# michaelneale/p2p-llm-tunnel

Measured on AMD Instinct MI355X. Metric: tunneled req/s + added p50 TTFT vs direct, mock-LLM SSE at 1/2/4/8 streams, higher is better.
Workload: dtype n/a

## Files before the change

### native/core/buf.h

```cpp
#pragma once

#include <atomic>
#include <cstdint>
#include <cstring>
#include <memory>
#include <string>
#include <string_view>
#include <vector>

namespace p2pt {

class Bytes {
 public:
  Bytes() = default;

  static Bytes copy(const void* p, size_t n) {
    auto v = std::make_shared<std::vector<uint8_t>>(static_cast<const uint8_t*>(p),
                                                    static_cast<const uint8_t*>(p) + n);
    return Bytes(std::move(v));
  }
  static Bytes copy(std::string_view s) { return copy(s.data(), s.size()); }
  static Bytes take(std::vector<uint8_t>&& v) {
    return Bytes(std::make_shared<std::vector<uint8_t>>(std::move(v)));
  }
// ... 61 lines not shown
    if (n < max_keep_) {
      bufs_.insert(bufs_.begin() + long(next_ < n ? next_ : n), b);
      next_ = next_ < n ? next_ + 1 : 0;
    }
    return b;
  }
  size_t size() const { return bufs_.size(); }

 private:
  static constexpr size_t kScan = 16;
  size_t size_, max_keep_;
  std::vector<RawBufPtr> bufs_;
  size_t next_ = 0;
};

inline Bytes slab_copy(const void* p, size_t n) {
  constexpr size_t kBlock = 64 * 1024, kMax = 2048;
  if (n == 0 || n > kMax) return Bytes::copy(p, n);
  struct Slab {
    BufPool pool{kBlock, 64};
    RawBufPtr cur;
    size_t off = kBlock;
  };
  thread_local Slab s;
  if (s.off + n > kBlock) {
    s.cur.reset();
    s.cur = s.pool.get();
    s.off = 0;
  }
  uint8_t* d = s.cur->data.get() + s.off;
  memcpy(d, p, n);
  s.off += (n + 15) & ~size_t(15);
  return Bytes::adopt(s.cur, d, n);
}

class ByteWriter {
 public:
  explicit ByteWriter(std::vector<uint8_t>& out) : out_(out) {}
  void u8(uint8_t v) { out_.push_back(v); }
  void u16(uint16_t v) {
    out_.push_back(uint8_t(v >> 8));
    out_.push_back(uint8_t(v));
  }
  void u32(uint32_t v) {
    out_.push_back(uint8_t(v >> 24));
    out_.push_back(uint8_t(v >> 16));
    out_.push_back(uint8_t(v >> 8));
    out_.push_back(uint8_t(v));
// ... 71 lines not shown
```

### native/http/client.cc

```cpp
#include "http/client.h"

#include "core/log.h"

#include <deque>

namespace p2pt::http {

using WarmWaiter = std::function<bool(std::shared_ptr<TcpConn>, const std::string&)>;

class ClientConnPool : public std::enable_shared_from_this<ClientConnPool> {
 public:
  explicit ClientConnPool(Reactor& r) : r_(r) {}
  std::shared_ptr<TcpConn> take(const std::string& key) {
    auto it = idle_.find(key);
    while (it != idle_.end() && !it->second.empty()) {
      auto c = it->second.back();
      it->second.pop_back();
      if (!c->closed()) return c;
    }
    return nullptr;
  }

  struct Warm {
    std::string host;
// ... 311 lines not shown
  live_calls()[this] = shared_from_this();
  pool_key_ = url_.scheme + "://" + url_.host + ":" + std::to_string(url_.port);
  pool_->call_started(pool_key_);
  counted_ = true;
  chunked_body_ = req_.stream_body && req_.content_length < 0;
  if (req_.stream_body) {
    for (auto& b : req_.body) queued_body_ += b.size();
    std::weak_ptr<ClientCall> w = shared_from_this();
    TcpConn::connect(*r_, url_.host, url_.port, url_.tls(), [w](std::shared_ptr<TcpConn> c, std::string e) {
      auto self = w.lock();
      if (!self || self->finished_) {
        if (c) c->close();
        return;
      }
      if (!c) {
        if (self->cb_.on_connect_failed) self->cb_.on_connect_failed();
        self->finish("error sending request for url (" + self->req_.url + "): " + e);
        return;
      }
      self->attach(c, false);
    });
    return;
  }
  if (auto c = pool_->take(pool_key_)) {
    attach(c, true);
    return;
  }
  if (auto c = pool_->take_warm(pool_key_)) {
    attach(c, true);
    return;
  }
  std::weak_ptr<ClientCall> w = shared_from_this();
  auto deliver = [w](std::shared_ptr<TcpConn> c, const std::string& e) -> bool {
    auto self = w.lock();
    if (!self || self->finished_) return false;
    if (!c) {
      if (self->cb_.on_connect_failed) self->cb_.on_connect_failed();
      self->finish("error sending request for url (" + self->req_.url + "): " + e);
      return true;
    }
    self->attach(c, false);
    return true;
  };
  if (pool_->wait_warm(pool_key_, deliver)) return;
  TcpConn::connect(*r_, url_.host, url_.port, url_.tls(), [deliver](std::shared_ptr<TcpConn> c, std::string e) {
    if (!deliver(c, e) && c) c->close();
  });
}

void ClientCall::attach(std::shared_ptr<TcpConn> c, bool reused) {
  conn_ = std::move(c);
  reused_ = reused;
  std::weak_ptr<ClientCall> w = shared_from_this();
  conn_->on_data([w](const uint8_t* p, size_t n) {
    if (auto s = w.lock()) s->on_data(p, n);
  });
  conn_->on_close([w](const std::string& err) {
    if (auto s = w.lock()) s->on_close(err);
  });
  std::string head;
  head.reserve(256);
  head += req_.method;
// ... 121 lines not shown

void ClientCall::on_close(const std::string& err) {
  auto self = shared_from_this();
  conn_.reset();
  if (finished_) return;
  if (!got_any_ && reused_) {
    reused_ = false;
    std::weak_ptr<ClientCall> w = self;
    TcpConn::connect(*r_, url_.host, url_.port, url_.tls(), [w](std::shared_ptr<TcpConn> c, std::string e) {
      auto s = w.lock();
      if (!s || s->finished_) {
        if (c) c->close();
        return;
      }
      if (!c) {
        if (s->cb_.on_connect_failed) s->cb_.on_connect_failed();
        s->finish("error sending request for url (" + s->req_.url + "): " + e);
        return;
      }
      s->attach(c, false);
    });
    return;
  }
  keep_alive_ = false;
  if (!head_done_) {
    process();
    if (finished_) return;
    finish("error sending request for url (" + req_.url + "): " +
           (err.empty() ? std::string("connection closed before message completed") : err));
    return;
  }
  paused_ = false;
// ... 92 lines not shown
```

### native/http/client.h

```cpp
#pragma once

#include <functional>
#include <map>
#include <memory>
#include <string>
#include <vector>

#include "core/net.h"
#include "http/http.h"

namespace p2pt::http {

struct ClientRequest {
  std::string method;
  std::string url;
  std::vector<Header> headers;
  std::vector<Bytes> body;
  uint64_t body_len = 0;
  bool force_content_length = false;
  bool stream_body = false;
  int64_t content_length = -1;
};

struct ClientCallbacks {
  std::function<void(bool reused)> on_sent;
  std::function<void(const Head&)> on_head;
  std::function<void(Bytes)> on_data;
  std::function<void(const std::string& err, bool before_head)> on_done;
  std::function<void()> on_connect_failed;
  std::function<void()> on_body_drain;
  size_t body_low_water = 64 * 1024;
};

class ClientConnPool;

class ClientCall : public std::enable_shared_from_this<ClientCall> {
 public:
  void pause();
  void resume();
  void cancel();
  bool finished() const { return finished_; }
  void write_body(Bytes b);
  void end_body();
  size_t body_backlog() const;
  ~ClientCall();

 private:
  friend class HttpClient;
  void start();
  void attach(std::shared_ptr<TcpConn> c, bool reused);
  void on_data(const uint8_t* p, size_t n);
  void on_close(const std::string& err);
  void finish(const std::string& err);
  void process();

  Reactor* r_ = nullptr;
  std::shared_ptr<ClientConnPool> pool_;
  ClientRequest req_;
  ClientCallbacks cb_;
  Url url_;
  std::string pool_key_;
  std::shared_ptr<TcpConn> conn_;
  bool reused_ = false;
  bool got_any_ = false;
  bool head_done_ = false;
  bool finished_ = false;
  bool paused_ = false;
  bool keep_alive_ = false;
// ... 27 lines not shown
```

### native/proto/frame.cc

```cpp
#include "proto/frame.h"

#include <algorithm>
#include <cstdlib>

#include <algorithm>
#include <cstring>

#include "core/crypto.h"

namespace p2pt::proto {

std::optional<MsgType> msg_type_from_u8(uint8_t v) {
  switch (v) {
    case 1: case 2: case 3: case 4:
    case 10: case 11: case 12: case 13: case 14: case 15:
    case 20: case 21: case 22:
    case 99:
      return MsgType(v);
    default:
      return std::nullopt;
  }
}

const char* msg_type_name(MsgType t) {
// ... 300 lines not shown
  }
  uint32_t st = 0;
  if (!get_u32(j, "stream_id", out.stream_id, err) || !get_u32(j, "status", st, err) ||
      !get_headers(j, out.headers, err))
    return false;
  if (st > 65535) {
    if (err) *err = "status out of range";
    return false;
  }
  out.status = uint16_t(st);
  return true;
}

Frame make_hello(const Hello& h) { return json_frame(MsgType::Hello, 0, h.to_json()); }
Frame make_agree(const Agree& a) { return json_frame(MsgType::Agree, 0, a.to_json()); }
Frame make_req_headers(const RequestHeaders& h) { return json_frame(MsgType::ReqHeaders, h.stream_id, h.to_json()); }
Frame make_res_headers(const ResponseHeaders& h) { return json_frame(MsgType::ResHeaders, h.stream_id, h.to_json()); }
Frame make_body(MsgType t, uint32_t sid, Bytes data) { return Frame{t, sid, std::move(data)}; }
Frame make_empty(MsgType t, uint32_t sid) { return Frame{t, sid, Bytes()}; }
Frame make_error(uint32_t sid, const std::string& msg) { return Frame{MsgType::Error, sid, Bytes::copy(msg)}; }
Frame make_credit(uint32_t sid, uint32_t bytes) {
  uint8_t b[4];
  wr32(b, bytes);
  return Frame{MsgType::Credit, sid, slab_copy(b, 4)};
}
uint32_t credit_bytes(const Frame& f) { return f.payload.size() == 4 ? rd32(f.payload.data()) : 0; }

static std::string trim_trailing_slashes(const std::string& s) {
  size_t n = s.size();
  while (n > 0 && s[n - 1] == '/') n--;
  return s.substr(0, n);
}
// ... 41 lines not shown
```

### native/proto/frame.h

```cpp
#pragma once

#include <cstdint>
#include <map>
#include <optional>
#include <string>
#include <vector>

#include "core/buf.h"
#include "core/json.h"

namespace p2pt::proto {

constexpr uint32_t kProtocolVersion = 1;
constexpr const char* kProtocolName = "httptunnel";
constexpr size_t kMaxFrameSize = 64 * 1024;
constexpr size_t kMaxBodyChunk = kMaxFrameSize - 128;
constexpr size_t kHeaderLen = 5;

enum class MsgType : uint8_t {
  Hello = 1,
  Agree = 2,
  Ping = 3,
  Pong = 4,
  ReqHeaders = 10,
// ... 69 lines not shown
  std::string method;
  std::string path;
  HeaderMap headers;
  Json to_json() const;
  static bool from_json(const Json& j, RequestHeaders& out, std::string* err);
};

struct ResponseHeaders {
  uint32_t stream_id = 0;
  uint16_t status = 200;
  HeaderMap headers;
  Json to_json() const;
  static bool from_json(const Json& j, ResponseHeaders& out, std::string* err);
};

Frame make_hello(const Hello& h);
Frame make_agree(const Agree& a);
Frame make_req_headers(const RequestHeaders& h);
Frame make_res_headers(const ResponseHeaders& h);
Frame make_body(MsgType t, uint32_t stream_id, Bytes data);
Frame make_empty(MsgType t, uint32_t stream_id);
Frame make_error(uint32_t stream_id, const std::string& msg);
Frame make_credit(uint32_t stream_id, uint32_t bytes);
uint32_t credit_bytes(const Frame& f);

constexpr int64_t kFlowWindow = 256 * 1024;
inline int64_t flow_window() { return kFlowWindow; }
constexpr size_t kFlowGrantMin = 16 * 1024;

constexpr int64_t kFlowMaxWindow = 8 * 1024 * 1024;
// ... 17 lines not shown
```

### native/py/module.cc

```cpp
#include <pybind11/pybind11.h>
#include <pybind11/stl.h>

#include "core/crypto.h"
#include "core/json.h"
#include "http/http.h"
#include "proto/frame.h"
#include "tunnel/app.h"
#include "ws/ws.h"

namespace py = pybind11;
using namespace p2pt;

static py::bytes to_py(const Bytes& b) { return py::bytes(reinterpret_cast<const char*>(b.data()), b.size()); }

static std::string canonical_json(const std::string& s) {
  Json j;
  std::string err;
  if (!Json::parse(s, j, &err)) throw py::value_error(err);
  return j.dump();
}

PYBIND11_MODULE(_native, m) {
  m.doc() = "p2p_llm_tunnel_amd native core";
  m.attr("MAX_FRAME_SIZE") = proto::kMaxFrameSize;
// ... 42 lines not shown
  });
  m.def("parse_request_headers", [](const std::string& s) {
    Json j;
    std::string err;
    proto::RequestHeaders h;
    if (!Json::parse(s, j, &err) || !proto::RequestHeaders::from_json(j, h, &err)) throw py::value_error(err);
    return py::make_tuple(h.stream_id, h.method, h.path, h.headers);
  });
  m.def("parse_response_headers", [](const std::string& s) {
    Json j;
    std::string err;
    proto::ResponseHeaders h;
    if (!Json::parse(s, j, &err) || !proto::ResponseHeaders::from_json(j, h, &err)) throw py::value_error(err);
    return py::make_tuple(h.stream_id, h.status, h.headers);
  });
  m.def("build_upstream_url", &proto::build_upstream_url);
  m.def("canonical_json", &canonical_json);
  m.def("crc32c", [](py::bytes b) {
    std::string s = b;
    return crc32c(s.data(), s.size());
  });
  m.def("crc32", [](py::bytes b) {
    std::string s = b;
    return crc32_ieee(s.data(), s.size());
  });
  m.def("ws_accept_key", [](const std::string& k) { return ws::accept_key(k); });
  m.def("ws_encode_frame", [](int op, py::bytes payload, bool mask) {
    std::string p = payload;
    return py::bytes(ws::encode_frame(ws::Op(op), p, mask));
  });
// ... 30 lines not shown
```

### native/tunnel/proxy.cc

```cpp
#include "tunnel/proxy.h"

#include <algorithm>
#include <cstdio>

#include "core/crypto.h"
#include "core/log.h"
#include "core/net.h"
#include "http/http.h"
#include "tunnel/assoc.h"
#include "tunnel/metrics.h"

namespace p2pt {

static const char* kT = "tunnel::proxy";

class ProxyWorker : public std::enable_shared_from_this<ProxyWorker> {
 public:
  ProxyWorker(Reactor& r, Reactor& assoc, std::weak_ptr<ProxySession> sess,
              std::shared_ptr<ProxySession::Shared> shared, size_t index)
      : r_(r), assoc_(assoc), sess_(std::move(sess)), shared_(std::move(shared)), index_(index) {}
  ~ProxyWorker();
  void init() {
    std::weak_ptr<ProxySession> w = sess_;
    size_t k = index_;
// ... 296 lines not shown
      body_.reset(mode, len);
      state_ = State::ReadingBody;
      reject_not_ready_ = true;
      if (body_.done()) finish_request_body();
      return true;
    }
    sid_ = sess->next_stream_id();
    metrics::counter_add("tunnel_streams_opened_total");
    trace::event("proxy", sid_, "accept");
    if (adopted_us_) {
      if (accepted_us_) trace::event_at("proxy", sid_, "tcp_accept", accepted_us_);
      trace::event_at("proxy", sid_, "conn_adopt", adopted_us_);
      accepted_us_ = adopted_us_ = 0;
    }
    if (req_.method == "GET") trace::event("proxy", sid_, "get");
    std::string path = req_.target;
    if (path.rfind("http://", 0) == 0 || path.rfind("https://", 0) == 0) {
      size_t s = path.find('/', path.find("://") + 3);
      path = s == std::string::npos ? "/" : path.substr(s);
    } else if (path == "*") {
      path = "/";
    }
    proto::RequestHeaders rh;
    rh.stream_id = sid_;
    rh.method = req_.method;
    rh.path = path;
    for (auto& hd : req_.headers)
      if (http::is_visible_ascii(hd.value)) proto::header_set(rh.headers, http::to_lower(hd.name), hd.value);
    LOG_DEBUG(kT, "proxying %s %s (stream %u)", rh.method.c_str(), rh.path.c_str(), sid_);
    proto::Frame hf = proto::make_req_headers(rh);
    if (hf.wire_size() > proto::kMaxFrameSize) {
      simple_and_close(431, "text/plain", "Request header fields too large for the tunnel");
      return false;
    }
    send_credit_ = proto::flow_window();
    credit_paused_ = false;
    owed_ = 0;
    rwin_ = proto::FlowWindow{};
    sess->register_stream(sid_, weak_from_this());
    stream_registered_ = true;
    sess->send(std::move(hf));
    if (req_.version_minor >= 1 && req_.has_token("expect", "100-continue"))
      conn_->write(std::string("HTTP/1.1 100 Continue\r\n\r\n"));
    body_.reset(mode, len);
    state_ = State::ReadingBody;
// ... 824 lines not shown
    }
    if (sched_->stream_queued(sid) <= cfg_.stream_budget / 4) {
      it->second.paused = false;
      p = paused_.erase(p);
      command(it->second.thread, Cmd{Cmd::Resume, sid});
      continue;
    }
    ++p;
  }
}

void ProxySession::route(const proto::Frame& f) {
  using proto::MsgType;
  switch (f.type) {
    case MsgType::ResHeaders: {
      Json j;
      std::string err;
      auto rh = std::make_shared<proto::ResponseHeaders>();
      if (!proto::json_parse_bytes(f.payload, j, &err) || !proto::ResponseHeaders::from_json(j, *rh, &err)) {
        LOG_ERROR(kT, "failed to parse response headers: %s", err.c_str());
        return;
      }
      LOG_DEBUG(kT, "response headers for stream %u: status=%u", rh->stream_id, rh->status);
      uint32_t sid = rh->stream_id;
      auto it = routes_.find(sid);
      if (it != routes_.end()) {
        Cmd c{Cmd::Headers, sid};
        c.urgent = true;
        c.rh = std::move(rh);
        command(it->second.thread, std::move(c));
      }
      break;
    }
    case MsgType::ResBody: {
// ... 181 lines not shown
```

### native/tunnel/serve.cc

```cpp
#include "tunnel/serve.h"

#include <algorithm>

#include "core/crypto.h"
#include "core/log.h"
#include "tunnel/assoc.h"
#include "tunnel/metrics.h"

namespace p2pt {

static const char* kT = "tunnel::serve";

class ServeWorker : public std::enable_shared_from_this<ServeWorker> {
 public:
  ServeWorker(Reactor& r, Reactor& assoc, std::weak_ptr<ServeSession> sess, const ServeConfig& cfg,
              std::vector<std::string> upstreams, bool is_inline)
      : r_(r), assoc_(assoc), sess_(std::move(sess)), cfg_(cfg), upstreams_(std::move(upstreams)),
        inline_(is_inline) {}

  ~ServeWorker() {
    auto calls = std::move(calls_);
    for (auto& kv : calls)
      if (kv.second.call) kv.second.call->cancel();
    client_.reset();
// ... 83 lines not shown
    if (f.type == proto::MsgType::ResBody && f.more.empty()) f.payload = out_->stage(f.payload);
    ev.frame = std::move(f);
    out_->push(std::move(ev), urgent);
  }

  void simple_response(uint32_t sid, uint16_t status, const std::string& body) {
    proto::ResponseHeaders rh;
    rh.stream_id = sid;
    rh.status = status;
    rh.headers.emplace_back("content-type", "text/plain");
    emit(sid, proto::make_res_headers(rh));
    emit(sid, proto::make_body(proto::MsgType::ResBody, sid, Bytes::copy(body)));
    emit(sid, proto::make_empty(proto::MsgType::ResEnd, sid));
  }

  void start(uint32_t sid, http::ClientRequest req, size_t body_chunk, bool retryable, bool grant) {
    if (!inline_) prewarm();
    std::weak_ptr<ServeWorker> w = shared_from_this();
    http::ClientCallbacks cb;
    if (req.stream_body) {
      cb.on_body_drain = [w, sid] {
        auto s = w.lock();
        if (!s) return;
        auto it = s->calls_.find(sid);
        if (it != s->calls_.end()) s->maybe_grant(sid, it->second);
      };
    }
    std::shared_ptr<ServeSession::Unreachable> back;
    if (retryable) {
      back = std::make_shared<ServeSession::Unreachable>();
      back->req = req;
    }
    auto unreachable = std::make_shared<bool>(false);
    cb.on_connect_failed = [unreachable] { *unreachable = true; };
    cb.on_sent = [sid](bool) { trace::event("serve", sid, "upstream_sent"); };
    cb.on_head = [w, sid](const http::Head& h) {
      auto s = w.lock();
      if (!s) return;
      proto::ResponseHeaders rh;
      rh.stream_id = sid;
      rh.status = uint16_t(h.status);
      for (auto& hd : h.headers)
        if (http::is_visible_ascii(hd.value)) proto::header_set(rh.headers, http::to_lower(hd.name), hd.value);
      s->emit(sid, proto::make_res_headers(rh), true);
      trace::event("serve", sid, "res_headers");
    };
    auto first = std::make_shared<bool>(true);
    size_t cs = body_chunk ? body_chunk : proto::kMaxBodyChunk;
    cb.on_data = [w, sid, first, cs](Bytes chunk) {
      auto s = w.lock();
      if (!s) return;
      const bool urgent = *first;
      if (*first) {
        *first = false;
        trace::event("serve", sid, "first_body");
      }
      size_t n = chunk.size();
      for (size_t off = 0; off < n; off += cs)
        s->emit(sid, proto::make_body(proto::MsgType::ResBody, sid, chunk.slice(off, cs)), urgent && off + cs >= n);
    };
    cb.on_done = [w, sid, back, unreachable](const std::string& err, bool before_head) {
      auto s = w.lock();
      if (!s) return;
      auto it = s->calls_.find(sid);
      if (it == s->calls_.end()) return;
      s->calls_.erase(it);
      ServeSession::Ev done(ServeSession::Ev::Done, sid);
      done.responded = !before_head;
      if (*unreachable && before_head) {
        if (back) {
          back->err = err;
          done.unreachable = back;
          s->out_->push(std::move(done));
          return;
        }
        done.unreachable = std::make_shared<ServeSession::Unreachable>();
        done.unreachable->err = err;
      }
      if (!err.empty() && before_head) {
        LOG_ERROR(kT, "upstream request failed: %s", err.c_str());
        metrics::counter_add("tunnel_upstream_errors_total");
        s->simple_response(sid, 502, "Bad Gateway: " + err);
      } else {
        if (!err.empty()) {
          LOG_ERROR(kT, "upstream stream error for stream %u: %s", sid, err.c_str());
          s->emit(sid, proto::make_error(sid, "upstream error: " + err));
        }
        s->emit(sid, proto::make_empty(proto::MsgType::ResEnd, sid));
        trace::event("serve", sid, "res_end");
        LOG_DEBUG(kT, "response %u complete", sid);
      }
      s->out_->push(std::move(done));
// ... 290 lines not shown
  sched_->send(proto::make_empty(proto::MsgType::Ping, 0));
  LOG_DEBUG(kT, "sent keepalive ping");
  std::weak_ptr<ServeSession> w = shared_from_this();
  ping_timer_ = r_.call_later_ms(cfg_.ping_interval_ms, [w] {
    if (auto s = w.lock()) {
      s->ping_timer_ = 0;
      s->send_ping();
    }
  });
}

void ServeSession::handle_frame(const proto::Frame& f) {
  using proto::MsgType;
  switch (f.type) {
    case MsgType::ReqHeaders: {
      Json j;
      std::string err;
      proto::RequestHeaders h;
      if (!proto::json_parse_bytes(f.payload, j, &err) || !proto::RequestHeaders::from_json(j, h, &err)) {
        LOG_WARN(kT, "malformed REQ_HEADERS for stream %u: %s", f.stream_id, err.c_str());
        send_simple_response(f.stream_id, 400, "Bad Request: malformed request headers");
        return;
      }
      LOG_DEBUG(kT, "request %u %s %s", h.stream_id, h.method.c_str(), h.path.c_str());
      trace::event("serve", h.stream_id, "req_headers");
      trace::rx_stamps("serve", h.stream_id);
      uint32_t sid = h.stream_id;
      Pending p;
      if (const std::string* cl = proto::header_get(h.headers, "content-length")) {
        char* end = nullptr;
        unsigned long long v = strtoull(cl->c_str(), &end, 10);
        if (end && *end == 0 && !cl->empty()) p.declared = int64_t(v);
      }
      p.headers = std::move(h);
// ... 184 lines not shown
  it->second.body_len = 0;
  send_simple_response(sid, 413, "Payload Too Large");
}

void ServeSession::start_request(uint32_t sid, Pending p, bool streaming) {
  if (!valid_method(p.headers.method)) {
    LOG_ERROR(kT, "failed to handle request: invalid HTTP method");
    send_simple_response(sid, 400, "Bad Request: invalid HTTP method");
    return;
  }
  if (inflight_.count(sid)) {
    LOG_WARN(kT, "stream %u reused while its response is in flight; ignoring the new request", sid);
    return;
  }
  http::ClientRequest req;
  req.method = p.headers.method;
  LOG_DEBUG(kT, "forwarding %s %s", p.headers.method.c_str(), p.headers.path.c_str());
  bool had_cl = false;
  for (auto& kv : p.headers.headers) {
    const std::string& k = kv.first;
    if (http::iequals(k, "host") || http::iequals(k, "connection") || http::iequals(k, "transfer-encoding"))
      continue;
    if (http::iequals(k, "content-length")) {
      had_cl = true;
      continue;
    }
    req.headers.push_back(http::Header{k, kv.second});
  }
  req.body = std::move(p.body);
  req.body_len = p.body_len;
  req.force_content_length = had_cl;
  if (streaming) {
    req.stream_body = true;
    req.content_length = p.declared;
  }
  metrics::counter_add("tunnel_upstream_requests_total");
  Inflight& fl = inflight_[sid];
  fl.up = pick_upstream();
  fl.route = BulkRoutes::key(req.method, p.headers.path);
  fl.thread = place_->pick(p.body_len >= Placement::kBulkBytes || p.declared >= int64_t(Placement::kBulkBytes) ||
                           bulk_routes_.bulk(fl.route));
  fl.path = std::move(p.headers.path);
// ... 108 lines not shown
```

Before: 15.97.

## Replace JSON tree header encode/decode with direct streaming codec

Adds a hand-written header codec that writes request/response header frames straight into a slab-allocated buffer and parses them without building a JSON tree. The proxy and serve paths switch to it, avoiding intermediate map and Json allocations per request. The serve worker's per-call callback state is merged into one shared context, and the retry copy of the request is now moved in only on connect failure rather than copied up front. Risks include subtle output differences versus the old JSON serializer in duplicate handling and escaping, plus a large new parser surface.

```diff
diff --git a/native/bin/headerbench_main.cc b/native/bin/headerbench_main.cc
--- /dev/null
+++ b/native/bin/headerbench_main.cc
@@ -0,0 +1,106 @@
+#include <algorithm>
+#include <chrono>
+#include <cstdio>
+#include <vector>
+
+#include "core/json.h"
+#include "http/http.h"
+#include "proto/frame.h"
+
+using namespace p2pt;
+using Clock = std::chrono::steady_clock;
+
+namespace {
+
+constexpr int kIters = 200000, kRounds = 5;
+
+template <class F>
+double ns_per_call(F&& f) {
+  double best = 1e30;
+  for (int r = 0; r < kRounds; r++) {
+    auto t0 = Clock::now();
+    for (int i = 0; i < kIters; i++) f(uint32_t(i));
+    best = std::min(best, std::chrono::duration<double, std::nano>(Clock::now() - t0).count() / kIters);
+  }
+  return best;
+}
+
+size_t g_sink = 0;
+
+void run(const char* name, bool response, const std::vector<http::Header>& hs) {
+  const std::string method = "POST", path = "/v1/chat/completions";
+  auto tree_encode = [&](uint32_t sid) {
+    if (response) {
+      proto::ResponseHeaders rh;
+      rh.stream_id = sid;
+      rh.status = 200;
+      for (auto& hd : hs)
+        if (http::is_visible_ascii(hd.value)) proto::header_set(rh.headers, http::to_lower(hd.name), hd.value);
+      return Bytes::copy(rh.to_json().dump());
+    }
+    proto::RequestHeaders rh;
+    rh.stream_id = sid;
+    rh.method = method;
+    rh.path = path;
+    for (auto& hd : hs)
+      if (http::is_visible_ascii(hd.value)) proto::header_set(rh.headers, http::to_lower(hd.name), hd.value);
+    return Bytes::copy(rh.to_json().dump());
+  };
+  std::vector<proto::HeaderRef> refs;
+  auto direct_encode = [&](uint32_t sid) {
+    refs.clear();
+    for (auto& hd : hs) refs.push_back(proto::HeaderRef{hd.name, hd.value});
+    return response ? proto::write_res_headers(sid, 200, refs) : proto::write_req_headers(sid, method, path, refs);
+  };
+  auto tree_decode = [&](const Bytes& b) {
+    Json j;
+    std::string err;
+    if (response) {
+      proto::ResponseHeaders h;
+      if (proto::json_parse_bytes(b, j, &err) && proto::ResponseHeaders::from_json(j, h, &err)) g_sink += h.headers.size();
+    } else {
+      proto::RequestHeaders h;
+      if (proto::json_parse_bytes(b, j, &err) && proto::RequestHeaders::from_json(j, h, &err)) g_sink += h.headers.size();
+    }
+  };
+  auto direct_decode = [&](const Bytes& b) {
+    std::string err;
+    if (response) {
+      proto::ResponseHeaders h;
+      if (proto::read_res_headers(b.view(), h, &err)) g_sink += h.headers.size();
+    } else {
+      proto::RequestHeaders h;
+      if (proto::read_req_headers(b.view(), h, &err)) g_sink += h.headers.size();
+    }
+  };
+  if (!(tree_encode(7) == direct_encode(7))) {
+    fprintf(stderr, "%s: the two encoders disagree\n", name);
+    exit(1);
+  }
+  const Bytes frame = direct_encode(1234);
+  const double te = ns_per_call([&](uint32_t i) { g_sink += tree_encode(i).size(); });
+  const double de = ns_per_call([&](uint32_t i) { g_sink += direct_encode(i).size(); });
+  const double td = ns_per_call([&](uint32_t) { tree_decode(frame); });
+  const double dd = ns_per_call([&](uint32_t) { direct_decode(frame); });
+  printf("{\"frame\": \"%s\", \"headers\": %zu, \"payload_bytes\": %zu, \"tree_encode_ns\": %.0f, "
+         "\"direct_encode_ns\": %.0f, \"tree_decode_ns\": %.0f, \"direct_decode_ns\": %.0f, "
+         "\"tree_ns_per_frame\": %.0f, \"direct_ns_per_frame\": %.0f}\n",
+         name, hs.size(), frame.size(), te, de, td, dd, te + td, de + dd);
+}
+
+}
+
+int main() {
+  run("req_headers", false,
+      {{"Host", "127.0.0.1:8000"},
+       {"User-Agent", "p2pt-loadgen"},
+       {"Accept", "text/event-stream"},
+       {"Content-Type", "application/json"},
+       {"Content-Length", "118"}});
+  run("res_headers", true,
+      {{"Server", "p2pt-mock"},
+       {"Date", "Tue, 20 Oct 2026 12:00:00 GMT"},
+       {"Content-Type", "text/event-stream"},
+       {"Cache-Control", "no-cache"}});
+  return g_sink ? 0 : 1;
+}
diff --git a/native/core/buf.h b/native/core/buf.h
--- a/native/core/buf.h
+++ b/native/core/buf.h
@@ -99,9 +99,13 @@
   size_t next_ = 0;
 };
 
-inline Bytes slab_copy(const void* p, size_t n) {
+inline Bytes slab_alloc(size_t n, uint8_t** out) {
   constexpr size_t kBlock = 64 * 1024, kMax = 2048;
-  if (n == 0 || n > kMax) return Bytes::copy(p, n);
+  if (n == 0 || n > kMax) {
+    std::shared_ptr<uint8_t> big(new uint8_t[n ? n : 1], std::default_delete<uint8_t[]>());
+    *out = big.get();
+    return Bytes::adopt(big, big.get(), n);
+  }
   struct Slab {
     BufPool pool{kBlock, 64};
     RawBufPtr cur;
@@ -114,9 +118,17 @@
     s.off = 0;
   }
   uint8_t* d = s.cur->data.get() + s.off;
+  s.off += (n + 15) & ~size_t(15);
+  *out = d;
+  return Bytes::adopt(s.cur, d, n);
+}
+
+inline Bytes slab_copy(const void* p, size_t n) {
+  if (n == 0 || n > 2048) return Bytes::copy(p, n);
+  uint8_t* d;
+  Bytes b = slab_alloc(n, &d);
   memcpy(d, p, n);
-  s.off += (n + 15) & ~size_t(15);
-  return Bytes::adopt(s.cur, d, n);
+  return b;
 }
 
 class ByteWriter {
diff --git a/native/http/client.cc b/native/http/client.cc
--- a/native/http/client.cc
+++ b/native/http/client.cc
@@ -349,8 +349,7 @@
         return;
       }
       if (!c) {
-        if (self->cb_.on_connect_failed) self->cb_.on_connect_failed();
-        self->finish("error sending request for url (" + self->req_.url + "): " + e);
+        self->connect_failed(e);
         return;
       }
       self->attach(c, false);
@@ -370,8 +369,7 @@
     auto self = w.lock();
     if (!self || self->finished_) return false;
     if (!c) {
-      if (self->cb_.on_connect_failed) self->cb_.on_connect_failed();
-      self->finish("error sending request for url (" + self->req_.url + "): " + e);
+      self->connect_failed(e);
       return true;
     }
     self->attach(c, false);
@@ -381,6 +379,12 @@
   TcpConn::connect(*r_, url_.host, url_.port, url_.tls(), [deliver](std::shared_ptr<TcpConn> c, std::string e) {
     if (!deliver(c, e) && c) c->close();
   });
+}
+
+void ClientCall::connect_failed(const std::string& e) {
+  std::string msg = "error sending request for url (" + req_.url + "): " + e;
+  if (cb_.on_connect_failed) cb_.on_connect_failed(std::move(req_));
+  finish(msg);
 }
 
 void ClientCall::attach(std::shared_ptr<TcpConn> c, bool reused) {
@@ -532,8 +536,7 @@
         return;
       }
       if (!c) {
-        if (s->cb_.on_connect_failed) s->cb_.on_connect_failed();
-        s->finish("error sending request for url (" + s->req_.url + "): " + e);
+        s->connect_failed(e);
         return;
       }
       s->attach(c, false);
diff --git a/native/http/client.h b/native/http/client.h
--- a/native/http/client.h
+++ b/native/http/client.h
@@ -27,7 +27,7 @@
   std::function<void(const Head&)> on_head;
   std::function<void(Bytes)> on_data;
   std::function<void(const std::string& err, bool before_head)> on_done;
-  std::function<void()> on_connect_failed;
+  std::function<void(ClientRequest&&)> on_connect_failed;
   std::function<void()> on_body_drain;
   size_t body_low_water = 64 * 1024;
 };
@@ -52,6 +52,7 @@
   void on_data(const uint8_t* p, size_t n);
   void on_close(const std::string& err);
   void finish(const std::string& err);
+  void connect_failed(const std::string& err);
   void process();
 
   Reactor* r_ = nullptr;
diff --git a/native/proto/frame.cc b/native/proto/frame.cc
--- a/native/proto/frame.cc
+++ b/native/proto/frame.cc
@@ -7,6 +7,7 @@
 #include <cstring>
 
 #include "core/crypto.h"
+#include "proto/header_codec.h"
 
 namespace p2pt::proto {
 
@@ -338,8 +339,45 @@
 
 Frame make_hello(const Hello& h) { return json_frame(MsgType::Hello, 0, h.to_json()); }
 Frame make_agree(const Agree& a) { return json_frame(MsgType::Agree, 0, a.to_json()); }
-Frame make_req_headers(const RequestHeaders& h) { return json_frame(MsgType::ReqHeaders, h.stream_id, h.to_json()); }
-Frame make_res_headers(const ResponseHeaders& h) { return json_frame(MsgType::ResHeaders, h.stream_id, h.to_json()); }
+
+Bytes write_req_headers(uint32_t stream_id, std::string_view method, std::string_view path,
+                        std::span<const HeaderRef> headers, HeaderRules rules) {
+  using codec::Slip;
+  return rules == HeaderRules::Http ? codec::write_headers<Slip::None, true>(stream_id, method, path, -1, headers)
+                                    : codec::write_headers<Slip::None, false>(stream_id, method, path, -1, headers);
+}
+
+Bytes write_res_headers(uint32_t stream_id, uint16_t status, std::span<const HeaderRef> headers, HeaderRules rules) {
+  using codec::Slip;
+  return rules == HeaderRules::Http ? codec::write_headers<Slip::None, true>(stream_id, {}, {}, status, headers)
+                                    : codec::write_headers<Slip::None, false>(stream_id, {}, {}, status, headers);
+}
+
+bool read_req_headers(std::string_view payload, RequestHeaders& out, std::string* err) {
+  return codec::read_req<codec::Slip::None>(payload, out, err);
+}
+
+bool read_res_headers(std::string_view payload, ResponseHeaders& out, std::string* err) {
+  return codec::read_res<codec::Slip::None>(payload, out, err);
+}
+
+namespace {
+std::span<const HeaderRef> refs_of(const HeaderMap& h) {
+  thread_local std::vector<HeaderRef> refs;
+  refs.clear();
+  for (auto& kv : h) refs.push_back(HeaderRef{kv.first, kv.second});
+  return refs;
+}
+}
+
+Frame make_req_headers(const RequestHeaders& h) {
+  return Frame{MsgType::ReqHeaders, h.stream_id,
+               write_req_headers(h.stream_id, h.method, h.path, refs_of(h.headers), HeaderRules::Verbatim)};
+}
+Frame make_res_headers(const ResponseHeaders& h) {
+  return Frame{MsgType::ResHeaders, h.stream_id,
+               write_res_headers(h.stream_id, h.status, refs_of(h.headers), HeaderRules::Verbatim)};
+}
 Frame make_body(MsgType t, uint32_t sid, Bytes data) { return Frame{t, sid, std::move(data)}; }
 Frame make_empty(MsgType t, uint32_t sid) { return Frame{t, sid, Bytes()}; }
 Frame make_error(uint32_t sid, const std::string& msg) { return Frame{MsgType::Error, sid, Bytes::copy(msg)}; }
diff --git a/native/proto/frame.h b/native/proto/frame.h
--- a/native/proto/frame.h
+++ b/native/proto/frame.h
@@ -3,7 +3,9 @@
 #include <cstdint>
 #include <map>
 #include <optional>
+#include <span>
 #include <string>
+#include <string_view>
 #include <vector>
 
 #include "core/buf.h"
@@ -107,6 +109,20 @@
   static bool from_json(const Json& j, ResponseHeaders& out, std::string* err);
 };
 
+struct HeaderRef {
+  std::string_view name, value;
+};
+enum class HeaderRules {
+  Http,
+  Verbatim,
+};
+Bytes write_req_headers(uint32_t stream_id, std::string_view method, std::string_view path,
+                        std::span<const HeaderRef> headers, HeaderRules rules = HeaderRules::Http);
+Bytes write_res_headers(uint32_t stream_id, uint16_t status, std::span<const HeaderRef> headers,
+                        HeaderRules rules = HeaderRules::Http);
+bool read_req_headers(std::string_view payload, RequestHeaders& out, std::string* err);
+bool read_res_headers(std::string_view payload, ResponseHeaders& out, std::string* err);
+
 Frame make_hello(const Hello& h);
 Frame make_agree(const Agree& a);
 Frame make_req_headers(const RequestHeaders& h);
diff --git a/native/proto/header_codec.h b/native/proto/header_codec.h
--- /dev/null
+++ b/native/proto/header_codec.h
@@ -0,0 +1,532 @@
+#pragma once
+
+#include <cstdint>
+#include <cstring>
+#include <span>
+#include <string>
+#include <string_view>
+#include <vector>
+
+#include "core/buf.h"
+#include "proto/frame.h"
+
+namespace p2pt::proto::codec {
+
+enum class Slip {
+  None,
+  WriterKeepsCase,
+  WriterHeadersFirst,
+  ReaderFirstDuplicate,
+  ReaderStatus65536,
+};
+
+
+inline char ascii_lower(char c) { return c >= 'A' && c <= 'Z' ? char(c + 32) : c; }
+
+inline bool visible_ascii(std::string_view v) {
+  for (unsigned char c : v)
+    if (!((c >= 32 && c < 127) || c == '\t')) return false;
+  return true;
+}
+
+inline size_t escaped_size(std::string_view s) {
+  size_t n = s.size() + 2;
+  for (unsigned char c : s) {
+    if (c >= 0x20 && c != '"' && c != '\\') continue;
+    switch (c) {
+      case '"': case '\\': case '\n': case '\r': case '\t': case '\b': case '\f': n += 1; break;
+      default: n += 5;
+    }
+  }
+  return n;
+}
+
+template <bool Lower>
+inline uint8_t* put_escaped(uint8_t* o, std::string_view s) {
+  static const char* hex = "0123456789abcdef";
+  *o++ = '"';
+  for (char ch : s) {
+    unsigned char c = static_cast<unsigned char>(ch);
+    if (c >= 0x20 && c != '"' && c != '\\') {
+      *o++ = uint8_t(Lower ? ascii_lower(ch) : ch);
+      continue;
+    }
+    *o++ = '\\';
+    switch (c) {
+      case '"': *o++ = '"'; break;
+      case '\\': *o++ = '\\'; break;
+      case '\n': *o++ = 'n'; break;
+      case '\r': *o++ = 'r'; break;
+      case '\t': *o++ = 't'; break;
+      case '\b': *o++ = 'b'; break;
+      case '\f': *o++ = 'f'; break;
+      default:
+        *o++ = 'u';
+        *o++ = '0';
+        *o++ = '0';
+        *o++ = uint8_t(hex[c >> 4]);
+        *o++ = uint8_t(hex[c & 15]);
+    }
+  }
+  *o++ = '"';
+  return o;
+}
+
+inline size_t u32_digits(uint32_t v) {
+  size_t n = 1;
+  while (v >= 10) {
+    v /= 10;
+    n++;
+  }
+  return n;
+}
+
+inline uint8_t* put_u32(uint8_t* o, uint32_t v) {
+  size_t n = u32_digits(v);
+  for (size_t i = n; i-- > 0; v /= 10) o[i] = uint8_t('0' + v % 10);
+  return o + n;
+}
+
+inline uint8_t* put_lit(uint8_t* o, std::string_view s) {
+  memcpy(o, s.data(), s.size());
+  return o + s.size();
+}
+
+template <bool Fold>
+inline bool same_name(std::string_view a, std::string_view b) {
+  if (a.size() != b.size()) return false;
+  if constexpr (!Fold) return a == b;
+  for (size_t i = 0; i < a.size(); i++)
+    if (ascii_lower(a[i]) != ascii_lower(b[i])) return false;
+  return true;
+}
+
+template <bool Fold>
+inline void plan_headers(std::span<const HeaderRef> h, int32_t* emit) {
+  const size_t n = h.size();
+  for (size_t i = 0; i < n; i++) emit[i] = (!Fold || visible_ascii(h[i].value)) ? int32_t(i) : -1;
+  for (size_t i = 0; i < n; i++) {
+    if (emit[i] < 0) continue;
+    for (size_t k = i + 1; k < n; k++) {
+      if (emit[k] < 0 || !same_name<Fold>(h[i].name, h[k].name)) continue;
+      emit[i] = emit[k];
+      emit[k] = -1;
+    }
+  }
+}
+
+template <Slip S, bool Fold>
+inline Bytes write_headers(uint32_t stream_id, std::string_view method, std::string_view path, int status,
+                           std::span<const HeaderRef> h) {
+  constexpr bool kLower = Fold && S != Slip::WriterKeepsCase;
+  constexpr size_t kInline = 32;
+  int32_t inline_emit[kInline];
+  std::vector<int32_t> heap_emit;
+  int32_t* emit = inline_emit;
+  if (h.size() > kInline) {
+    heap_emit.resize(h.size());
+    emit = heap_emit.data();
+  }
+  plan_headers<Fold>(h, emit);
+
+  constexpr std::string_view kSid = "{\"stream_id\":", kMethod = ",\"method\":", kPath = ",\"path\":",
+                             kStatus = ",\"status\":", kHeaders = ",\"headers\":{";
+  size_t n = kSid.size() + u32_digits(stream_id) + kHeaders.size() + 2;
+  if (status < 0) n += kMethod.size() + escaped_size(method) + kPath.size() + escaped_size(path);
+  else n += kStatus.size() + u32_digits(uint32_t(status));
+  size_t members = 0;
+  for (size_t i = 0; i < h.size(); i++) {
+    if (emit[i] < 0) continue;
+    n += escaped_size(h[i].name) + 1 + escaped_size(h[size_t(emit[i])].value);
+    members++;
+  }
+  if (members) n += members - 1;
+
+  uint8_t* o;
+  Bytes out = slab_alloc(n, &o);
+  [[maybe_unused]] const uint8_t* const begin = o;
+  auto put_header_members = [&] {
+    o = put_lit(o, kHeaders);
+    bool first = true;
+    for (size_t i = 0; i < h.size(); i++) {
+      if (emit[i] < 0) continue;
+      if (!first) *o++ = ',';
+      first = false;
+      o = put_escaped<kLower>(o, h[i].name);
+      *o++ = ':';
+      o = put_escaped<false>(o, h[size_t(emit[i])].value);
+    }
+    *o++ = '}';
+  };
+  o = put_lit(o, kSid);
+  o = put_u32(o, stream_id);
+  if (status < 0) {
+    o = put_lit(o, kMethod);
+    o = put_escaped<false>(o, method);
+    if constexpr (S == Slip::WriterHeadersFirst) put_header_members();
+    o = put_lit(o, kPath);
+    o = put_escaped<false>(o, path);
+    if constexpr (S != Slip::WriterHeadersFirst) put_header_members();
+  } else {
+    o = put_lit(o, kStatus);
+    o = put_u32(o, uint32_t(status));
+    put_header_members();
+  }
+  *o++ = '}';
+  if (size_t(o - begin) != n) __builtin_trap();
+  return out;
+}
+
+
+template <Slip S>
+struct Reader {
+  const char* p;
+  const char* end;
+  const char* err = nullptr;
+  const char* field = nullptr;
+  int depth = 0;
+  std::string key;
+
+  enum class Slot : uint8_t { Absent, Ok, Bad };
+
+  Reader(std::string_view text) : p(text.data()), end(text.data() + text.size()) {}
+
+  bool fail(const char* m) {
+    if (!err) err = m;
+    return false;
+  }
+  void ws() {
+    while (p < end && (*p == ' ' || *p == '\t' || *p == '\n' || *p == '\r')) p++;
+  }
+  static void utf8(std::string* o, uint32_t cp) {
+    if (!o) return;
+    if (cp < 0x80) o->push_back(char(cp));
+    else if (cp < 0x800) {
+      o->push_back(char(0xC0 | (cp >> 6)));
+      o->push_back(char(0x80 | (cp & 0x3F)));
+    } else if (cp < 0x10000) {
+      o->push_back(char(0xE0 | (cp >> 12)));
+      o->push_back(char(0x80 | ((cp >> 6) & 0x3F)));
+      o->push_back(char(0x80 | (cp & 0x3F)));
+    } else {
+      o->push_back(char(0xF0 | (cp >> 18)));
+      o->push_back(char(0x80 | ((cp >> 12) & 0x3F)));
+      o->push_back(char(0x80 | ((cp >> 6) & 0x3F)));
+      o->push_back(char(0x80 | (cp & 0x3F)));
+    }
+  }
+  bool hex4(uint32_t& v) {
+    if (end - p < 4) return fail("truncated \\u escape");
+    v = 0;
+    for (int i = 0; i < 4; i++) {
+      char c = *p++;
+      v <<= 4;
+      if (c >= '0' && c <= '9') v |= uint32_t(c - '0');
+      else if (c >= 'a' && c <= 'f') v |= uint32_t(c - 'a' + 10);
+      else if (c >= 'A' && c <= 'F') v |= uint32_t(c - 'A' + 10);
+      else return fail("bad \\u escape");
+    }
+    return true;
+  }
+  bool string(std::string* o) {
+    if (p >= end || *p != '"') return fail("expected string");
+    p++;
+    while (true) {
+      const char* s = p;
+      while (p < end && *p != '"' && *p != '\\' && static_cast<unsigned char>(*p) >= 0x20) p++;
+      if (o) o->append(s, size_t(p - s));
+      if (p >= end) return fail("unterminated string");
+      char c = *p++;
+      if (c == '"') return true;
+      if (c != '\\') return fail("control character in string");
+      if (p >= end) return fail("unterminated escape");
+      char e = *p++;
+      char plain = 0;
+      switch (e) {
+        case '"': plain = '"'; break;
+        case '\\': plain = '\\'; break;
+        case '/': plain = '/'; break;
+        case 'b': plain = '\b'; break;
+        case 'f': plain = '\f'; break;
+        case 'n': plain = '\n'; break;
+        case 'r': plain = '\r'; break;
+        case 't': plain = '\t'; break;
+        case 'u': {
+          uint32_t cp;
+          if (!hex4(cp)) return false;
+          if (cp >= 0xD800 && cp < 0xDC00) {
+            uint32_t lo;
+            if (end - p >= 6 && p[0] == '\\' && p[1] == 'u') {
+              p += 2;
+              if (!hex4(lo)) return false;
+              if (lo >= 0xDC00 && lo < 0xE000) cp = 0x10000 + ((cp - 0xD800) << 10) + (lo - 0xDC00);
+              else {
+                utf8(o, 0xFFFD);
+                cp = lo;
+              }
+            } else cp = 0xFFFD;
+          } else if (cp >= 0xDC00 && cp < 0xE000) cp = 0xFFFD;
+          utf8(o, cp);
+          continue;
+        }
+        default: return fail("bad escape");
+      }
+      if (o) o->push_back(plain);
+    }
+  }
+  bool number(bool* is_u32, uint32_t* v) {
+    bool is_float = false, neg = false, big = false;
+    uint64_t acc = 0;
+    auto digit = [&](char c) {
+      if (big) return;
+      acc = acc * 10 + uint64_t(c - '0');
+      if (acc > UINT32_MAX) big = true;
+    };
+    if (p < end && *p == '-') {
+      neg = true;
+      p++;
+    }
+    if (p >= end || !(*p >= '0' && *p <= '9')) return fail("bad number");
+    if (*p == '0') p++;
+    else while (p < end && *p >= '0' && *p <= '9') digit(*p++);
+    if (p < end && *p == '.') {
+      is_float = true;
+      p++;
+      if (p >= end || !(*p >= '0' && *p <= '9')) return fail("bad number");
+      while (p < end && *p >= '0' && *p <= '9') p++;
+    }
+    if (p < end && (*p == 'e' || *p == 'E')) {
+      is_float = true;
+      p++;
+      if (p < end && (*p == '+' || *p == '-')) p++;
+      if (p >= end || !(*p >= '0' && *p <= '9')) return fail("bad number");
+      while (p < end && *p >= '0' && *p <= '9') p++;
+    }
+    if (is_u32) {
+      *is_u32 = !is_float && !big && !(neg && acc != 0);
+      *v = uint32_t(acc);
+    }
+    return true;
+  }
+  bool lit(const char* w) {
+    size_t n = strlen(w);
+    if (size_t(end - p) < n || memcmp(p, w, n) != 0) return fail("bad literal");
+    p += n;
+    return true;
+  }
+  bool skip_value() {
+    if (++depth > 128) return fail("nesting too deep");
+    ws();
+    if (p >= end) return fail("unexpected end");
+    bool ok = true;
+    switch (*p) {
+      case '{': {
+        p++;
+        ws();
+        if (p < end && *p == '}') {
+          p++;
+          break;
+        }
+        while (true) {
+          ws();
+          if (!string(nullptr)) return false;
+          ws();
+          if (p >= end || *p != ':') return fail("expected ':'");
+          p++;
+          if (!skip_value()) return false;
+          ws();
+          if (p < end && *p == ',') { p++; continue; }
+          if (p < end && *p == '}') { p++; break; }
+          return fail("expected ',' or '}'");
+        }
+        break;
+      }
+      case '[': {
+        p++;
+        ws();
+        if (p < end && *p == ']') {
+          p++;
+          break;
+        }
+        while (true) {
+          if (!skip_value()) return false;
+          ws();
+          if (p < end && *p == ',') { p++; continue; }
+          if (p < end && *p == ']') { p++; break; }
+          return fail("expected ',' or ']'");
+        }
+        break;
+      }
+      case '"': ok = string(nullptr); break;
+      case 't': ok = lit("true"); break;
+      case 'f': ok = lit("false"); break;
+      case 'n': ok = lit("null"); break;
+      default: ok = number(nullptr, nullptr);
+    }
+    depth--;
+    return ok;
+  }
+
+  bool u32_member(Slot& slot, uint32_t& out) {
+    if (S == Slip::ReaderFirstDuplicate && slot != Slot::Absent) return skip_value();
+    ws();
+    if (p >= end) return fail("unexpected end");
+    switch (*p) {
+      case '{': case '[': case '"': case 't': case 'f': case 'n':
+        slot = Slot::Bad;
+        return skip_value();
+    }
+    bool is_u32 = false;
+    uint32_t v = 0;
+    if (!number(&is_u32, &v)) return false;
+    slot = is_u32 ? Slot::Ok : Slot::Bad;
+    if (is_u32) out = v;
+    return true;
+  }
+  bool string_member(Slot& slot, std::string& out) {
+    if (S == Slip::ReaderFirstDuplicate && slot != Slot::Absent) return skip_value();
+    ws();
+    if (p < end && *p == '"') {
+      slot = Slot::Ok;
+      out.clear();
+      return string(&out);
+    }
+    slot = Slot::Bad;
+    return skip_value();
+  }
+  bool headers_member(Slot& slot, HeaderMap& out) {
+    if (S == Slip::ReaderFirstDuplicate && slot != Slot::Absent) return skip_value();
+    ws();
+    if (p >= end || *p != '{') {
+      slot = Slot::Bad;
+      return skip_value();
+    }
+    out.clear();
+    std::vector<uint8_t> not_string;
+    depth++;
+    p++;
+    ws();
+    if (p < end && *p == '}') {
+      p++;
+    } else {
+      while (true) {
+        ws();
+        key.clear();
+        if (!string(&key)) return false;
+        ws();
+        if (p >= end || *p != ':') return fail("expected ':'");
+        p++;
+        size_t idx = 0;
+        while (idx < out.size() && out[idx].first != key) idx++;
+        if (idx == out.size()) out.emplace_back(std::move(key), std::string());
+        ws();
+        if (p < end && *p == '"') {
+          out[idx].second.clear();
+          if (!string(&out[idx].second)) return false;
+          if (idx < not_string.size()) not_string[idx] = 0;
+        } else {
+          if (!skip_value()) return false;
+          if (not_string.size() <= idx) not_string.resize(idx + 1, 0);
+          not_string[idx] = 1;
+        }
+        ws();
+        if (p < end && *p == ',') { p++; continue; }
+        if (p < end && *p == '}') { p++; break; }
+        return fail("expected ',' or '}'");
+      }
+    }
+    depth--;
+    slot = Slot::Ok;
+    for (uint8_t b : not_string)
+      if (b) slot = Slot::Bad;
+    return true;
+  }
+
+  template <class Member>
+  bool document(Member member) {
+    depth = 1;
+    ws();
+    if (p >= end) return fail("unexpected end");
+    if (*p != '{') return fail("expected object");
+    p++;
+    ws();
+    if (p < end && *p == '}') {
+      p++;
+    } else {
+      while (true) {
+        ws();
+        key.clear();
+        if (!string(&key)) return false;
+        ws();
+        if (p >= end || *p != ':') return fail("expected ':'");
+        p++;
+        int r = member(std::string_view(key));
+        if (r == 0 || (r < 0 && !skip_value())) return false;
+        ws();
+        if (p < end && *p == ',') { p++; continue; }
+        if (p < end && *p == '}') { p++; break; }
+        return fail("expected ',' or '}'");
+      }
+    }
+    ws();
+    if (p != end) return fail("trailing characters");
+    return true;
+  }
+
+  bool require(Slot s, const char* missing, const char* invalid) {
+    if (s == Slot::Ok) return true;
+    if (!field) field = s == Slot::Absent ? missing : invalid;
+    return false;
+  }
+  void report(std::string_view text, std::string* out) const {
+    if (!out) return;
+    if (err) *out = std::string(err) + " at offset " + std::to_string(p - text.data());
+    else *out = field ? field : "invalid header frame";
+  }
+};
+
+template <Slip S>
+inline bool read_req(std::string_view text, RequestHeaders& out, std::string* err) {
+  using R = Reader<S>;
+  R r(text);
+  typename R::Slot sid = R::Slot::Absent, method = sid, path = sid, headers = sid;
+  bool ok = r.document([&](std::string_view k) -> int {
+    if (k == "stream_id") return r.u32_member(sid, out.stream_id);
+    if (k == "method") return r.string_member(method, out.method);
+    if (k == "path") return r.string_member(path, out.path);
+    if (k == "headers") return r.headers_member(headers, out.headers);
+    return -1;
+  });
+  ok = ok && r.require(sid, "missing field `stream_id`", "invalid type for field `stream_id`") &&
+       r.require(method, "missing field `method`", "invalid type for field `method`") &&
+       r.require(path, "missing field `path`", "invalid type for field `path`") &&
+       r.require(headers, "missing field `headers`", "invalid `headers`: an object of strings is expected");
+  if (!ok) r.report(text, err);
+  return ok;
+}
+
+template <Slip S>
+inline bool read_res(std::string_view text, ResponseHeaders& out, std::string* err) {
+  using R = Reader<S>;
+  R r(text);
+  typename R::Slot sid = R::Slot::Absent, status = sid, headers = sid;
+  uint32_t st = 0;
+  bool ok = r.document([&](std::string_view k) -> int {
+    if (k == "stream_id") return r.u32_member(sid, out.stream_id);
+    if (k == "status") return r.u32_member(status, st);
+    if (k == "headers") return r.headers_member(headers, out.headers);
+    return -1;
+  });
+  ok = ok && r.require(sid, "missing field `stream_id`", "invalid type for field `stream_id`") &&
+       r.require(status, "missing field `status`", "invalid type for field `status`") &&
+       r.require(headers, "missing field `headers`", "invalid `headers`: an object of strings is expected");
+  if (ok && st > (S == Slip::ReaderStatus65536 ? 65536u : 65535u)) {
+    r.field = "status out of range";
+    ok = false;
+  }
+  if (!ok) r.report(text, err);
+  else out.status = uint16_t(st);
+  return ok;
+}
+
+}
diff --git a/native/py/module.cc b/native/py/module.cc
--- a/native/py/module.cc
+++ b/native/py/module.cc
@@ -80,6 +80,33 @@
     if (!Json::parse(s, j, &err) || !proto::ResponseHeaders::from_json(j, h, &err)) throw py::value_error(err);
     return py::make_tuple(h.stream_id, h.status, h.headers);
   });
+  m.def("req_headers_frame", [](uint32_t sid, const std::string& method, const std::string& path,
+                                std::vector<std::pair<std::string, std::string>> headers, bool http_rules) {
+    std::vector<proto::HeaderRef> refs;
+    for (auto& kv : headers) refs.push_back(proto::HeaderRef{kv.first, kv.second});
+    auto rules = http_rules ? proto::HeaderRules::Http : proto::HeaderRules::Verbatim;
+    return to_py(proto::Frame{proto::MsgType::ReqHeaders, sid, proto::write_req_headers(sid, method, path, refs, rules)}
+                     .encode());
+  }, py::arg("stream_id"), py::arg("method"), py::arg("path"), py::arg("headers"), py::arg("http_rules") = false);
+  m.def("res_headers_frame", [](uint32_t sid, uint16_t status, std::vector<std::pair<std::string, std::string>> headers,
+                                bool http_rules) {
+    std::vector<proto::HeaderRef> refs;
+    for (auto& kv : headers) refs.push_back(proto::HeaderRef{kv.first, kv.second});
+    auto rules = http_rules ? proto::HeaderRules::Http : proto::HeaderRules::Verbatim;
+    return to_py(proto::Frame{proto::MsgType::ResHeaders, sid, proto::write_res_headers(sid, status, refs, rules)}.encode());
+  }, py::arg("stream_id"), py::arg("status"), py::arg("headers"), py::arg("http_rules") = false);
+  m.def("read_request_headers", [](py::bytes payload) {
+    std::string s = payload, err;
+    proto::RequestHeaders h;
+    if (!proto::read_req_headers(s, h, &err)) throw py::value_error(err);
+    return py::make_tuple(h.stream_id, h.method, h.path, h.headers);
+  });
+  m.def("read_response_headers", [](py::bytes payload) {
+    std::string s = payload, err;
+    proto::ResponseHeaders h;
+    if (!proto::read_res_headers(s, h, &err)) throw py::value_error(err);
+    return py::make_tuple(h.stream_id, h.status, h.headers);
+  });
   m.def("build_upstream_url", &proto::build_upstream_url);
   m.def("canonical_json", &canonical_json);
   m.def("crc32c", [](py::bytes b) {
diff --git a/native/tunnel/proxy.cc b/native/tunnel/proxy.cc
--- a/native/tunnel/proxy.cc
+++ b/native/tunnel/proxy.cc
@@ -334,21 +334,18 @@
       accepted_us_ = adopted_us_ = 0;
     }
     if (req_.method == "GET") trace::event("proxy", sid_, "get");
-    std::string path = req_.target;
+    std::string_view path = req_.target;
     if (path.rfind("http://", 0) == 0 || path.rfind("https://", 0) == 0) {
       size_t s = path.find('/', path.find("://") + 3);
-      path = s == std::string::npos ? "/" : path.substr(s);
+      path = s == std::string_view::npos ? std::string_view("/") : path.substr(s);
     } else if (path == "*") {
       path = "/";
     }
-    proto::RequestHeaders rh;
-    rh.stream_id = sid_;
-    rh.method = req_.method;
-    rh.path = path;
-    for (auto& hd : req_.headers)
-      if (http::is_visible_ascii(hd.value)) proto::header_set(rh.headers, http::to_lower(hd.name), hd.value);
-    LOG_DEBUG(kT, "proxying %s %s (stream %u)", rh.method.c_str(), rh.path.c_str(), sid_);
-    proto::Frame hf = proto::make_req_headers(rh);
+    LOG_DEBUG(kT, "proxying %s %.*s (stream %u)", req_.method.c_str(), int(path.size()), path.data(), sid_);
+    thread_local std::vector<proto::HeaderRef> refs;
+    refs.clear();
+    for (auto& hd : req_.headers) refs.push_back(proto::HeaderRef{hd.name, hd.value});
+    proto::Frame hf{proto::MsgType::ReqHeaders, sid_, proto::write_req_headers(sid_, req_.method, path, refs)};
     if (hf.wire_size() > proto::kMaxFrameSize) {
       simple_and_close(431, "text/plain", "Request header fields too large for the tunnel");
       return false;
@@ -1203,10 +1200,9 @@
   using proto::MsgType;
   switch (f.type) {
     case MsgType::ResHeaders: {
-      Json j;
       std::string err;
       auto rh = std::make_shared<proto::ResponseHeaders>();
-      if (!proto::json_parse_bytes(f.payload, j, &err) || !proto::ResponseHeaders::from_json(j, *rh, &err)) {
+      if (!proto::read_res_headers(f.payload.view(), *rh, &err)) {
         LOG_ERROR(kT, "failed to parse response headers: %s", err.c_str());
         return;
       }
diff --git a/native/tunnel/serve.cc b/native/tunnel/serve.cc
--- a/native/tunnel/serve.cc
+++ b/native/tunnel/serve.cc
@@ -121,68 +121,81 @@
     emit(sid, proto::make_empty(proto::MsgType::ResEnd, sid));
   }
 
+  struct CallCtx {
+    std::weak_ptr<ServeWorker> w;
+    uint32_t sid;
+    size_t chunk;
+    bool retryable;
+    bool unreachable = false;
+    bool first = true;
+    http::ClientRequest back;
+  };
+
   void start(uint32_t sid, http::ClientRequest req, size_t body_chunk, bool retryable, bool grant) {
     if (!inline_) prewarm();
-    std::weak_ptr<ServeWorker> w = shared_from_this();
+    auto owner = std::make_shared<CallCtx>();
+    CallCtx* c = owner.get();
+    c->w = weak_from_this();
+    c->sid = sid;
+    c->chunk = body_chunk ? body_chunk : proto::kMaxBodyChunk;
+    c->retryable = retryable;
     http::ClientCallbacks cb;
     if (req.stream_body) {
-      cb.on_body_drain = [w, sid] {
-        auto s = w.lock();
+      cb.on_body_drain = [c] {
+        auto s = c->w.lock();
         if (!s) return;
-        auto it = s->calls_.find(sid);
-        if (it != s->calls_.end()) s->maybe_grant(sid, it->second);
+        auto it = s->calls_.find(c->sid);
+        if (it != s->calls_.end()) s->maybe_grant(c->sid, it->second);
       };
     }
-    std::shared_ptr<ServeSession::Unreachable> back;
-    if (retryable) {
-      back = std::make_shared<ServeSession::Unreachable>();
-      back->req = req;
-    }
-    auto unreachable = std::make_shared<bool>(false);
-    cb.on_connect_failed = [unreachable] { *unreachable = true; };
-    cb.on_sent = [sid](bool) { trace::event("serve", sid, "upstream_sent"); };
-    cb.on_head = [w, sid](const http::Head& h) {
-      auto s = w.lock();
+    cb.on_connect_failed = [c](http::ClientRequest&& r) {
+      c->unreachable = true;
+      if (c->retryable) c->back = std::move(r);
+    };
+    cb.on_sent = [c](bool) { trace::event("serve", c->sid, "upstream_sent"); };
+    cb.on_head = [c](const http::Head& h) {
+      auto s = c->w.lock();
       if (!s) return;
-      proto::ResponseHeaders rh;
-      rh.stream_id = sid;
-      rh.status = uint16_t(h.status);
-      for (auto& hd : h.headers)
-        if (http::is_visible_ascii(hd.value)) proto::header_set(rh.headers, http::to_lower(hd.name), hd.value);
-      s->emit(sid, proto::make_res_headers(rh), true);
+      const uint32_t sid = c->sid;
+      thread_local std::vector<proto::HeaderRef> refs;
+      refs.clear();
+      for (auto& hd : h.headers) refs.push_back(proto::HeaderRef{hd.name, hd.value});
+      s->emit(sid, proto::Frame{proto::MsgType::ResHeaders, sid, proto::write_res_headers(sid, uint16_t(h.status), refs)},
+              true);
       trace::event("serve", sid, "res_headers");
     };
-    auto first = std::make_shared<bool>(true);
-    size_t cs = body_chunk ? body_chunk : proto::kMaxBodyChunk;
-    cb.on_data = [w, sid, first, cs](Bytes chunk) {
-      auto s = w.lock();
+    cb.on_data = [c](Bytes chunk) {
+      auto s = c->w.lock();
       if (!s) return;
-      const bool urgent = *first;
-      if (*first) {
-        *first = false;
+      const uint32_t sid = c->sid;
+      const size_t cs = c->chunk;
+      const bool urgent = c->first;
+      if (c->first) {
+        c->first = false;
         trace::event("serve", sid, "first_body");
       }
       size_t n = chunk.size();
       for (size_t off = 0; off < n; off += cs)
         s->emit(sid, proto::make_body(proto::MsgType::ResBody, sid, chunk.slice(off, cs)), urgent && off + cs >= n);
     };
-    cb.on_done = [w, sid, back, unreachable](const std::string& err, bool before_head) {
-      auto s = w.lock();
+    cb.on_done = [owner](const std::string& err, bool before_head) {
+      CallCtx* c = owner.get();
+      auto s = c->w.lock();
       if (!s) return;
+      const uint32_t sid = c->sid;
       auto it = s->calls_.find(sid);
       if (it == s->calls_.end()) return;
       s->calls_.erase(it);
       ServeSession::Ev done(ServeSession::Ev::Done, sid);
       done.responded = !before_head;
-      if (*unreachable && before_head) {
-        if (back) {
-          back->err = err;
-          done.unreachable = back;
+      if (c->unreachable && before_head) {
+        done.unreachable = std::make_shared<ServeSession::Unreachable>();
+        done.unreachable->err = err;
+        if (c->retryable) {
+          done.unreachable->req = std::move(c->back);
           s->out_->push(std::move(done));
           return;
         }
-        done.unreachable = std::make_shared<ServeSession::Unreachable>();
-        done.unreachable->err = err;
       }
       if (!err.empty() && before_head) {
         LOG_ERROR(kT, "upstream request failed: %s", err.c_str());
@@ -503,10 +516,9 @@
   using proto::MsgType;
   switch (f.type) {
     case MsgType::ReqHeaders: {
-      Json j;
       std::string err;
       proto::RequestHeaders h;
-      if (!proto::json_parse_bytes(f.payload, j, &err) || !proto::RequestHeaders::from_json(j, h, &err)) {
+      if (!proto::read_req_headers(f.payload.view(), h, &err)) {
         LOG_WARN(kT, "malformed REQ_HEADERS for stream %u: %s", f.stream_id, err.c_str());
         send_simple_response(f.stream_id, 400, "Bad Request: malformed request headers");
         return;
@@ -721,8 +733,9 @@
     return;
   }
   http::ClientRequest req;
-  req.method = p.headers.method;
   LOG_DEBUG(kT, "forwarding %s %s", p.headers.method.c_str(), p.headers.path.c_str());
+  req.method = std::move(p.headers.method);
+  req.headers.reserve(p.headers.headers.size());
   bool had_cl = false;
   for (auto& kv : p.headers.headers) {
     const std::string& k = kv.first;
@@ -732,7 +745,7 @@
       had_cl = true;
       continue;
     }
-    req.headers.push_back(http::Header{k, kv.second});
+    req.headers.push_back(http::Header{std::move(kv.first), std::move(kv.second)});
   }
   req.body = std::move(p.body);
   req.body_len = p.body_len;
```

New measurement: 15.97. No clear change (-0.0%).
